# openmm/NNPOps

Measured on AMD Instinct MI355X. Metric: AEV+forces evaluations/sec (ANI-2x symmetry functions, energy+gradient), 10k-atom periodic box, higher is better.
Workload: dtype f32

## Files before the change

### nnpops_amd/csrc/ani.hip

```cpp
#include <algorithm>
#include <cmath>
#include <cstdlib>
#include <cstring>
#include <vector>

#include "ani_kernels.h"
#include "ani_fallback_kernels.h"
#include "ani_angular_mfma.h"
#include "ani_angular_bwd.h"
#include "ani_angular_generic.h"
#include "ani_radial_bwd.h"
#include "ani_build_forward.h"
#include "ani_box_grad.h"
#include "host_common.h"

using namespace nnpops;

constexpr int kRbwdLatencyAtoms = 8192;
constexpr int kFuseAtoms = 4096;
struct nnpops_ani {
    AniParams hp{};
    AngularConsts ac{};
    AniParams* d_params = nullptr;
    int device = 0;
    hipStream_t stream = nullptr;
    int nfrp = 0, nfzp = 0;
    int algorithm = 0;
    int32_t* d_species = nullptr;
    int2* d_segment = nullptr;
    float4* d_nbr = nullptr;
    int* d_cnt_pos = nullptr;
    float4* d_recA = nullptr;
    float4* d_recB = nullptr;
    int* d_ids = nullptr;
// ... 3 lines not shown
    int* d_bucket_offsets = nullptr;
    bool chunked_forward = true;
    int forward_kernel = 2;
    bool generic = false;
    bool mfma_ok = false;
    bool fwd_identity = false;
    int fwd_chunk = 192;
    bool fwd_chunk_forced = false;
    int fwd_waves_per_atom = 2;
    bool backward_forced = false;
    bool fwd_uniform = false;
    bool fwd_grid = true;
    bool bwd_literal = true;
    bool fwd_literal = false;
    int fuse_forward = -1;
    bool rbwd_lanes = true;
    int scatter_mode = -1;
    bool scatter_now = false;
    bool last_fused_build = false;
    int last_bwd_mode = -1;
    int last_radial_lanes = -1;
    int last_tile = -1;
    int last_compact = -1;
    bool fine_grid = true;
    bool fwd_row_via_lds = true;
    int fwd_occ = 7;
    bool fwd_dynamic = false;
    int nstreams = 1;
    hipStream_t side[3] = {nullptr, nullptr, nullptr};
    hipEvent_t ev_fork = nullptr, ev_join[3] = {nullptr, nullptr, nullptr};
// ... 5 lines not shown
    int fwd_atoms_per_group = 1;
    int* d_cnt_a = nullptr;
    int* d_cnt_ro = nullptr;
    double* d_box_partials = nullptr;
    int* d_status = nullptr;
    int* h_status = nullptr;
    int* h_status_dev = nullptr;
    int check_stamp = 0;
    bool check_pending = false;
    CellGrid* d_grid = nullptr;
    int* d_cell_count = nullptr;
    int* d_cell_start = nullptr;
    int* d_atom_cell = nullptr;
    int* d_atom_rank = nullptr;
    int* d_sorted_cell = nullptr;
    int* d_tile_total = nullptr;
    int* d_unsorted_atom = nullptr;
    int* d_sorted_atom = nullptr;
    float4* d_sorted_pos = nullptr;
    int max_cells = 0;
    int* d_hist = nullptr;
    int* d_bins = nullptr;
    int bin_cap = 64;
    bool cells_disabled = false;
    int cap = 0;
    bool cap_fitted = false;
    int cap_angular = 0;
    int tile = 32;
    bool compact_bwd = false;
    bool computed = false;
// ... 304 lines not shown
        h->last_bwd_mode = 1;
        if (lb > 64 * 1024) NNPOPS_HIP_TRY(hipFuncSetAttribute((const void*)k, hipFuncAttributeMaxDynamicSharedMemorySize, (int)lb));
        hipLaunchKernelGGL(k, dim3(N), dim3(64), lb, sp.stream, h->d_params, h->ac, h->cap, h->cap_angular, h->cap_angular, h->d_recA, h->d_recB, h->d_tri,
                           h->d_cnt_a, h->d_cnt_ro, g, h->ld_angular, h->d_leg_force, h->d_centre_force, h->d_ids, nullptr, 0, h->hp.NB, (int)lb, nullptr, 0, N, 0);
    }
    NNPOPS_HIP_TRY(hipGetLastError());
    return NNPOPS_OK;
}

int dispatch_angular(nnpops_ani* h, bool forward, const float* g, float* out, const Span& sp) {
    KernelTimer timer(h, forward ? NNPOPS_ANI_K_ANGULAR_FWD : NNPOPS_ANI_K_ANGULAR_BWD, sp.stream);
    if (h->generic) return h->hp.torchani ? launch_generic<true>(h, forward, g, out, sp) : launch_generic<false>(h, forward, g, out, sp);
    return h->hp.torchani ? dispatch_factors<true>(h, forward, g, out, sp) : dispatch_factors<false>(h, forward, g, out, sp);
}

int fused_chunk(const nnpops_ani* h) {
    return forward_chunk(h, (size_t)h->cap_angular * 2 * sizeof(float4) + (size_t)triples_capacity(h->cap_angular) * sizeof(int) + 64, 12 * sizeof(float));
}

bool build_forward_fused(const nnpops_ani* h, const float* angular) {
    const bool want = h->fuse_forward < 0 ? h->hp.N <= kFuseAtoms : h->fuse_forward != 0;
    return want && !h->generic && h->forward_kernel == 2 && h->fwd_waves_per_atom == 2 && h->nfrp == 8 && h->nfzp == 4 &&
           h->nstreams == 1 && h->fwd_identity && h->ld_angular % 4 == 0 && ((uintptr_t)angular & 15) == 0 &&
           build_forward_lds_bytes<8, 4>(h->cap, h->cap_angular, h->hp.S, h->hp.NB, fused_chunk(h)) <= 160 * 1024;
}

template <bool TA>
int launch_build_forward(nnpops_ani* h, const BuildInputs& in, const BuildOutputs& out, float* angular, const Span& sp) {
    int tri_offset = 0;
    const int CH = fused_chunk(h);
    const size_t lds = (build_forward_lds_bytes<8, 4>(h->cap, h->cap_angular, h->hp.S, h->hp.NB, CH, &tri_offset) + 15) & ~(size_t)15;
    const int vec_ok = 1 | (h->store_mode << 1) | (h->fwd_row_via_lds ? 8 : 0);
    const bool uni = h->fwd_uniform && h->fwd_grid && h->hp.nFR == 8 && h->hp.nFZ == 4;
    const bool dyn = h->fwd_dynamic && h->fwd_row_via_lds && h->hp.NB <= 63 && h->hp.NB * h->hp.nA <= CH * 12;
    auto k = h->fwd_occ == 6 ? ani_build_forward<TA, 8, 4, 6>
           : dyn ? (uni ? ani_build_forward<TA, 8, 4, 7, 1, true> : ani_build_forward<TA, 8, 4, 7, 0, true>)
           : uni ? ani_build_forward<TA, 8, 4, 7, 1> : ani_build_forward<TA, 8, 4, 7>;
    if (uni && h->fwd_literal && h->fwd_occ != 6) k = dyn ? ani_build_forward<TA, 8, 4, 7, 2, true> : ani_build_forward<TA, 8, 4, 7, 2>;
    if (lds > 64 * 1024) NNPOPS_HIP_TRY(hipFuncSetAttribute((const void*)k, hipFuncAttributeMaxDynamicSharedMemorySize, (int)lds));
    hipLaunchKernelGGL(k, dim3(sp.nw), dim3(128), lds, sp.stream, h->d_params, in, out, h->cap, h->cap_angular, CH, angular,
                       h->ld_angular, vec_ok, tri_offset, sp.w0, sp.nw);
    NNPOPS_HIP_TRY(hipGetLastError());
    return NNPOPS_OK;
}

bool pair_backward_fits(const nnpops_ani* h) {
// ... 52 lines not shown
    NNPOPS_REQUIRE(radial_cutoff > 0 && angular_cutoff > 0, "cutoffs must be positive");
    NNPOPS_REQUIRE(angular_cutoff <= radial_cutoff,
                   "angular cutoff (%g) must not exceed the radial cutoff (%g): angular neighbours are drawn from the radial scan "
                   "(reference CpuANISymmetryFunctions.cpp:129-135)", angular_cutoff, radial_cutoff);
    NNPOPS_REQUIRE(num_radial > 0 && num_radial <= kMaxRadialFns, "num_radial must be in [1, %d]", kMaxRadialFns);
    NNPOPS_REQUIRE(num_angular > 0 && num_angular <= kMaxAngularFns, "num_angular must be in [1, %d]", kMaxAngularFns);
    NNPOPS_REQUIRE(atom_species && radial_eta_rs && angular_eta_rs_zeta_ths, "NULL parameter array");
    for (int i = 0; i < num_atoms; i++)
        NNPOPS_REQUIRE(atom_species[i] >= 0 && atom_species[i] < num_species, "atom_species[%d] = %d is outside [0, %d)", i,
                       atom_species[i], num_species);
    int ndev = 0;
    if (hipGetDeviceCount(&ndev) != hipSuccess || ndev == 0) return fail(NNPOPS_ERR_NO_DEVICE, "no HIP device available");
    NNPOPS_REQUIRE(device >= 0 && device < ndev, "device %d out of range (have %d)", device, ndev);

    nnpops_ani* h = new nnpops_ani();
    AniParams& hp = h->hp;
    hp.N = num_atoms; hp.S = num_species; hp.nR = num_radial; hp.nA = num_angular;
    hp.NB = num_species * (num_species + 1) / 2;
    hp.periodic = periodic != 0; hp.torchani = torchani != 0;
    hp.rcr = radial_cutoff; hp.rca = angular_cutoff;
    hp.rcr2 = radial_cutoff * radial_cutoff; hp.rca2 = angular_cutoff * angular_cutoff;
    hp.radial_scale = torchani ? 0.25f : 1.0f;
    hp.inv_rcr = 1.0f / radial_cutoff; hp.inv_rca = 1.0f / angular_cutoff;
    hp.kp_shift = 0;
    while ((1 << hp.kp_shift) < num_radial) hp.kp_shift++;
    hp.angle_damp = torchani ? 0.95f : 1.0f;
    for (int k = 0; k < num_radial; k++) {
        hp.rad_eta[k] = radial_eta_rs[2 * k];
        hp.rad_rs[k] = radial_eta_rs[2 * k + 1];
        hp.rad_c[k] = -radial_eta_rs[2 * k] * kLog2e;
// ... 61 lines not shown
            for (size_t b = 0; b < live.size(); b++)
                for (int p = 0; p < hp.fwd_split; p++) hp.fwd_slot_bucket[b * hp.fwd_split + p] = live[b];
        }
        for (int c = 0; c < kMaxAngularFns; c++) hp.m_of_c[c] = -1;
        h->fwd_identity = num_angular == h->nfrp * h->nfzp;
        for (int m = 0; m < num_angular; m++) {
            hp.m_of_c[hp.c_of_m[m]] = m;
            if (hp.c_of_m[m] != m) h->fwd_identity = false;
        }
        hp.fwd_zero_shift = 0;
        while ((4 << hp.fwd_zero_shift) < num_angular && hp.fwd_zero_shift < 6) hp.fwd_zero_shift++;
        h->fwd_identity = h->fwd_identity && num_angular <= 256;
        h->forward_kernel = h->mfma_ok ? 2 : -1;
        if (const char* e = std::getenv("NNPOPS_ANI_FWD_CHUNK")) { h->fwd_chunk = std::min(512, std::max(64, (std::atoi(e) + 15) / 16 * 16)); h->fwd_chunk_forced = true; }
        if (const char* e = std::getenv("NNPOPS_ANI_FUSE")) h->fuse_forward = std::atoi(e) != 0 ? 1 : 0;
        if (const char* e = std::getenv("NNPOPS_ANI_LPT")) h->lpt = std::atoi(e);
        if (const char* e = std::getenv("NNPOPS_ANI_CELL_ATOMS")) h->cell_atoms = std::max(1, std::atoi(e));
        if (const char* e = std::getenv("NNPOPS_ANI_RBWD")) h->rbwd_lanes = std::atoi(e) != 0;
        if (const char* e = std::getenv("NNPOPS_ANI_SCATTER")) h->scatter_mode = std::atoi(e) != 0 ? 1 : 0;
        if (const char* e = std::getenv("NNPOPS_ANI_FINE_GRID")) h->fine_grid = std::atoi(e) != 0;
        if (const char* e = std::getenv("NNPOPS_ANI_FWD_ROWLDS")) h->fwd_row_via_lds = std::atoi(e) != 0;
        if (const char* e = std::getenv("NNPOPS_ANI_FWD_OCC")) h->fwd_occ = std::atoi(e);
        {
            std::vector<double> frac(num_species, 0.0);
            for (int i = 0; i < num_atoms; i++) frac[atom_species[i]] += 1.0 / num_atoms;
            double fmax = 0;
            for (int a = 0; a < num_species; a++)
                for (int b = a; b < num_species; b++) fmax = std::max(fmax, frac[a] * frac[b] * (a == b ? 1.0 : 2.0));
            h->fwd_dynamic = h->mfma_ok && 32.0 * fmax / hp.fwd_split > 3.0;
        }
// ... 25 lines not shown
    if (periodic && (rc = dev_alloc(&h->d_box_partials, (size_t)9 * ani_box_blocks(num_atoms)))) return cleanup(rc);
    if ((rc = alloc_rows(h))) return cleanup(rc);
    h->max_cells = num_atoms + 4096;
    if ((rc = dev_alloc(&h->d_grid, 1))) return cleanup(rc);
    if ((rc = dev_alloc(&h->d_cell_count, (size_t)h->max_cells))) return cleanup(rc);
    if ((rc = dev_alloc(&h->d_cell_start, (size_t)h->max_cells + 1))) return cleanup(rc);
    if (const char* e = std::getenv("NNPOPS_CELL_BIN_CAP")) h->bin_cap = std::max(4, std::atoi(e) & ~3);
    if (periodic && num_atoms <= kBinnedAtoms) {
        if ((rc = dev_alloc(&h->d_hist, (size_t)kHistWords))) return cleanup(rc);
        if ((rc = dev_alloc(&h->d_bins, (size_t)kBinnedCells * h->bin_cap))) return cleanup(rc);
        if (hipMemset(h->d_hist, 0, sizeof(int) * kHistWords) != hipSuccess) return cleanup(fail(NNPOPS_ERR_HIP, "memset failed"));
    }
    if ((rc = dev_alloc(&h->d_atom_cell, (size_t)num_atoms))) return cleanup(rc);
    if ((rc = dev_alloc(&h->d_atom_rank, (size_t)num_atoms))) return cleanup(rc);
    if ((rc = dev_alloc(&h->d_sorted_cell, (size_t)num_atoms))) return cleanup(rc);
    if ((rc = dev_alloc(&h->d_tile_total, (size_t)h->max_cells / kScanTile + 2))) return cleanup(rc);
    if ((rc = dev_alloc(&h->d_sorted_atom, (size_t)num_atoms))) return cleanup(rc);
    if ((rc = dev_alloc(&h->d_work_order, (size_t)num_atoms))) return cleanup(rc);
    if ((rc = dev_alloc(&h->d_class_tile, (size_t)num_atoms))) return cleanup(rc);
    if (hipMemset(h->d_class_tile, 255, (size_t)num_atoms) != hipSuccess) return cleanup(fail(NNPOPS_ERR_HIP, "memset failed"));
    hp.class_tile = h->d_class_tile;
    if (const char* e = std::getenv("NNPOPS_ANI_BWD_CLASSES")) h->bwd_by_class = std::atoi(e) != 0;
    if (const char* e = std::getenv("NNPOPS_ANI_BWD_CLASS_MIN")) h->bwd_class_min = std::max(0, std::atoi(e));
    if (const char* e = std::getenv("NNPOPS_ANI_BWD_CLASS_ATOMS")) h->bwd_class_atoms = std::max(0, std::atoi(e));
    if ((rc = dev_alloc(&h->d_unsorted_atom, (size_t)num_atoms))) return cleanup(rc);
    if ((rc = dev_alloc(&h->d_sorted_pos, (size_t)num_atoms))) return cleanup(rc);
    if ((rc = dev_alloc(&h->d_bucket_offsets, (size_t)num_atoms * (hp.NB + 1)))) return cleanup(rc);
    hp.bucket_offsets = h->d_bucket_offsets;
    if (hipMemset(h->d_bucket_offsets, 0, sizeof(int) * (size_t)num_atoms * (hp.NB + 1)) != hipSuccess)
        return cleanup(fail(NNPOPS_ERR_HIP, "memset failed"));
// ... 35 lines not shown
        hipMemset(h->d_cnt_a, 0, sizeof(int) * num_atoms) != hipSuccess ||
        hipMemset(h->d_cnt_ro, 0, sizeof(int) * num_atoms) != hipSuccess || hipMemset(h->d_cnt_pos, 0, sizeof(int) * num_atoms) != hipSuccess)
        return cleanup(fail(NNPOPS_ERR_HIP, "parameter upload failed: %s", hipGetErrorString(hipGetLastError())));
    *out = h;
    return NNPOPS_OK;
}

int nnpops_ani_destroy(nnpops_ani_t h) {
    if (!h) return NNPOPS_OK;
    DeviceGuard guard(h->device);
    dev_free(h->d_params); dev_free(h->d_species); dev_free(h->d_segment);
    dev_free(h->d_nbr); dev_free(h->d_recA); dev_free(h->d_recB); dev_free(h->d_tri); dev_free(h->d_cnt_a); dev_free(h->d_cnt_ro); dev_free(h->d_cnt_pos); dev_free(h->d_status); dev_free(h->d_box_partials);
    dev_free(h->d_ids); dev_free(h->d_leg_force); dev_free(h->d_centre_force); dev_free(h->d_bucket_offsets);
    dev_free(h->d_hist); dev_free(h->d_bins);
    dev_free(h->d_grid); dev_free(h->d_cell_count); dev_free(h->d_cell_start); dev_free(h->d_atom_cell);
    dev_free(h->d_atom_rank); dev_free(h->d_sorted_cell); dev_free(h->d_tile_total); dev_free(h->d_sorted_atom); dev_free(h->d_work_order); dev_free(h->d_class_tile); dev_free(h->d_unsorted_atom); dev_free(h->d_sorted_pos);
    for (int q = 0; q < 3; q++) {
        if (h->side[q]) (void)hipStreamDestroy(h->side[q]);
        if (h->ev_join[q]) (void)hipEventDestroy(h->ev_join[q]);
    }
    if (h->ev_fork) (void)hipEventDestroy(h->ev_fork);
    if (h->h_status) (void)hipHostFree(h->h_status);
    for (int k = 0; k < NNPOPS_ANI_NUM_KERNELS; k++) {
        for (hipEvent_t e : h->ev_start[k]) (void)hipEventDestroy(e);
        for (hipEvent_t e : h->ev_stop[k]) (void)hipEventDestroy(e);
    }
    delete h;
    return NNPOPS_OK;
}

int nnpops_ani_set_stream(nnpops_ani_t h, void* stream) {
// ... 51 lines not shown
    DeviceGuard guard(h->device);
    if (!guard.ok) return fail(NNPOPS_ERR_HIP, "cannot select device %d", h->device);
    const int N = h->hp.N;
    const bool per = h->hp.periodic;

    const int lds_bw = (int)((builder_lds_bytes(h->cap, h->hp.S, h->hp.NB) + 15) & ~(size_t)15);
    const int wpg_b = waves_per_group(lds_bw);
    const size_t lds_b = (size_t)lds_bw * wpg_b;
    const dim3 ablock(64 * wpg_b);
    const bool use_cells = !h->d_segment && (h->algorithm == 2 || (h->algorithm == 0 && N >= h->cell_atoms && !h->cells_disabled));
    h->last_used_cells = use_cells;
    if (use_cells) {
        KernelTimer timer(h, NNPOPS_ANI_K_CELL_GRID);
        const CellBuffers cb{h->d_grid, h->d_cell_count, h->d_cell_start, h->d_atom_cell, h->d_atom_rank,
                             h->d_unsorted_atom, h->d_sorted_atom, h->d_sorted_pos, h->max_cells,
                             h->d_hist, h->d_bins, h->bin_cap, h->fine_grid ? 1 : 0, h->d_sorted_cell, h->d_tile_total};
        launch_cell_build(h->stream, N, positions, box, per, h->hp.rcr, h->d_species, cb);
    }
    h->can_split = !h->generic && h->forward_kernel == 2 && h->backward_kernel >= 1 &&
                   pair_backward_fits(h);
    Span spans[4];
    const int nspans = make_spans(h, spans);
    int rc = fork_streams(h, spans, nspans);
    if (rc != NNPOPS_OK) return rc;
    for (int q = 0; q < nspans; q++) {
        const Span& sp = spans[q];
        const dim3 sgrid(div_up(sp.nw, wpg_b));
        h->last_fused_build = build_forward_fused(h, angular);
        if (h->last_fused_build) {
            KernelTimer timer(h, NNPOPS_ANI_K_NEIGHBORS, sp.stream);
            KernelTimer merged_timer(h, NNPOPS_ANI_K_NEIGHBORS, sp.stream, true);
            const BuildInputs in{box, h->d_grid, h->d_cell_start, h->d_sorted_cell, h->d_sorted_pos, h->d_hist, positions, h->d_species,
                                 h->d_segment, use_cells ? 1 : 0, per ? 1 : 0};
            const BuildOutputs out{h->d_nbr, h->d_recA, h->d_recB, h->d_ids, h->d_tri, h->d_cnt_a, h->d_cnt_ro, h->d_cnt_pos, h->d_status, radial, h->ld_radial};
            rc = h->hp.torchani ? launch_build_forward<true>(h, in, out, angular, sp) : launch_build_forward<false>(h, in, out, angular, sp);
            if (rc != NNPOPS_OK) return rc;
            continue;
        }
        KernelTimer merged_timer(h, NNPOPS_ANI_K_NEIGHBORS, sp.stream, true);
        {
        KernelTimer timer(h, NNPOPS_ANI_K_NEIGHBORS, sp.stream);
        if (use_cells) {
            if (per)
                hipLaunchKernelGGL(ani_neighbors_cells<true>, sgrid, ablock, lds_b, sp.stream, h->d_params, box, h->d_grid,
                                   h->d_cell_start, h->d_sorted_cell, h->d_sorted_pos, h->d_nbr, h->cap, h->cap_angular, h->d_recA,
                                   h->d_recB, h->d_ids, h->d_tri, h->d_cnt_a, h->d_cnt_ro, h->d_cnt_pos, h->d_status, radial, h->ld_radial, lds_bw, h->d_hist,
                                   sp.w0, sp.nw);
            else
// ... 332 lines not shown
    if (!guard.ok) return fail(NNPOPS_ERR_HIP, "cannot select device %d", h->device);
    NNPOPS_HIP_TRY(hipMemcpyAsync(value, h->d_status + kStatOverflow, sizeof(int32_t), hipMemcpyDeviceToHost, h->stream));
    NNPOPS_HIP_TRY(hipStreamSynchronize(h->stream));
    return NNPOPS_OK;
}

int nnpops_ani_describe(nnpops_ani_t h, char* text, int capacity) {
    NNPOPS_REQUIRE(h != nullptr && text != nullptr && capacity > 0, "NULL argument");
    const bool uni = h->fwd_uniform && h->hp.nFR == h->nfrp && h->hp.nFZ == h->nfzp;
    const bool shape2x = h->nfrp == 8 && h->nfzp == 4;
    std::snprintf(text, (size_t)capacity,
                  "forward=%s backward=%d generic=%d uniform=%d grid=%d literal=%d dynamic_quads=%d fused_build=%d cap=%d cap_angular=%d "
                  "chunk=%d classes=%d cells=%d scatter=%d row_major_walk=%d bwd_mode=%d radial_bwd=%s tile=%d compact=%d",
                  h->forward_kernel == 2 ? "mfma" : h->forward_kernel == 1 ? "chunked" : "merge", h->backward_kernel, (int)h->generic,
                  (int)uni, (int)(uni && h->fwd_grid), (int)(uni && h->fwd_grid && shape2x && h->fwd_literal), (int)h->fwd_dynamic,
                  (int)(h->computed ? h->last_fused_build : (h->fuse_forward < 0 ? h->hp.N <= kFuseAtoms : h->fuse_forward != 0)), h->cap, h->cap_angular,
                  h->generic ? h->fwd_chunk : forward_chunk(h, (size_t)h->cap_angular * 2 * sizeof(float4), (size_t)(h->nfrp + h->nfzp) * sizeof(float)),
                  (int)h->bwd_classes.size(), (int)h->last_used_cells,
                  (int)h->scatter_now, h->hp.tri_row_major,
                  h->last_bwd_mode, h->last_radial_lanes < 0 ? "none" : h->last_radial_lanes ? "lanes" : "rows", h->last_tile, h->last_compact);
    return NNPOPS_OK;
}

int nnpops_ani_enable_timing(nnpops_ani_t h, int enable) {
    NNPOPS_REQUIRE(h != nullptr, "NULL handle");
    h->timing_mask = enable == 1 ? ~0u : (unsigned)enable >> 1;
    for (int k = 0; k < NNPOPS_ANI_NUM_KERNELS; k++) { h->ev_used[k] = 0; h->timing_seen[k] = 0; }
    return NNPOPS_OK;
}

int nnpops_ani_set_timing_stride(nnpops_ani_t h, int every) {
// ... 54 lines not shown
```

### nnpops_amd/csrc/ani_build_forward.h

```cpp
#pragma once

#include "ani_angular_mfma.h"

namespace nnpops {

template <int NFRP, int NFZP>
__host__ __device__ inline size_t build_forward_lds_bytes(int cap, int capA, int S, int NB, int CH, int* tri_offset = nullptr) {
    const size_t recs = (size_t)capA * 2 * sizeof(float4);
    const size_t staging = (size_t)(CH + 1) * (NFRP + NFZP) * sizeof(float) + 64 * sizeof(int);
    const size_t builder = ((builder_lds_bytes(cap, S, NB) + 15) & ~(size_t)15) + 32;
    const size_t mid = ((staging > builder ? staging : builder) + 15) & ~(size_t)15;
    if (tri_offset) *tri_offset = (int)(recs + mid);
    return recs + mid + (size_t)triples_capacity(capA) * sizeof(int);
}

struct BuildInputs {
    const float* box;
    const CellGrid* grid;
    const int* cell_start;
    const int* sorted_cell;
    const float4* sorted_pos;
    int* cell_hist;
    const float* pos;
    const int* species;
    const int2* segment;
    int use_cells, periodic;
};

struct BuildOutputs {
    float4* nbr;
    float4 *recA, *recB;
    int *ids, *tri, *cnt_a, *cnt_ro, *cnt_pos, *status;
    float* radial;
    int ld_radial;
};

template <bool TORCHANI, int NFRP, int NFZP, int OCC, int UNI = 0, bool DYN = false>
__global__ __launch_bounds__(128, OCC) void ani_build_forward(const AniParams* __restrict__ P, BuildInputs in, BuildOutputs out, int cap,
                                                              int capA, int CH, float* __restrict__ angular, int ld_angular,
                                                              int vec_ok, int tri_offset, int w0, int nw) {
    extern __shared__ __attribute__((aligned(16))) char lds_raw[];
    const int role = __builtin_amdgcn_readfirstlane(wave_in_group());
    const int lane = lane_id();
    float4* recA_l = (float4*)lds_raw;
    float4* recB_l = recA_l + capA;
    float4* stage = recB_l + capA;
    float* rscratch = (float*)(stage + cap);
    int* groups = (int*)(rscratch + 3 * cap + 64 * P->S);
    const AtomGroups G = carve_groups(groups, P->S, P->NB);
    int* shared = groups + ((group_ints(P->S, P->NB, cap) + 3) & ~(size_t)3);
    int* tri_l = (int*)(lds_raw + tri_offset);
    clear_cell_histogram(in.use_cells ? in.cell_hist : nullptr);

    const float rcr2 = P->rcr2, rca2 = P->rca2;
    Box b{};
    if (in.periodic) b = load_box(in.box);
    CellGrid g{};
    if (in.use_cells) g = *in.grid;

    {
        const int w = blockIdx.x;
        const int slot_id = w0 + w;
        int i = slot_id;
        float4 me = make_float4(0.f, 0.f, 0.f, 0.f);
        const bool void_grid = in.use_cells && !g.ok;
        if (in.use_cells && !void_grid) {
            me = in.sorted_pos[slot_id];
            i = __float_as_int(me.w) & kIdMask;
        } else if (!in.use_cells) {
            me = make_float4(in.pos[3 * i], in.pos[3 * i + 1], in.pos[3 * i + 2], 0.f);
        }
        if (role == 0) {
            int na = 0, nro = 0;
            if (void_grid) {
                if (lane == 0 && slot_id == 0) atomicOr(&out.status[kStatOverflow], g.bin_overflow ? 6 : 2);
            } else if (in.use_cells) {
                const int c = in.sorted_cell[slot_id];
                int cx, cy, cz;
                split_cell(g, c, cx, cy, cz);
                const WideStencil st = gather_wide_stencil(g, in.cell_start, cx, cy, cz);
// ... 49 lines not shown
        const int na_raw = shared[0], nro_raw = shared[1];
        clamp_counts(na_raw, nro_raw, cap, capA, n, nro_c);
        if (!void_grid) {
            if (role == 1) {
                flush_row(out.nbr + (size_t)slot_id * cap, stage, cap, na_raw, nro_raw);
                radial_forward_from_lds(P, stage, cap, n, nro_c, rscratch, out.radial + (size_t)i * out.ld_radial);
            } else {
                finalize_angular(P, stage, n, out.recA + (size_t)i * capA, out.recB + (size_t)i * capA, out.ids + (size_t)i * capA, capA,
                                 out.tri + (size_t)i * triples_capacity(capA), P->bucket_offsets + (size_t)i * (P->NB + 1), G,
                                 recA_l, recB_l, tri_l);
            }
        }
        __syncthreads();
        MfmaForward<TORCHANI, NFRP, NFZP, 2, UNI, DYN> F;
        F.init(P, capA, CH, vec_ok, angular, ld_angular, lds_raw, role);
        F.atom(i, n, [&](int t) { return tri_l[t]; }, [&](int bk) { return G.boff[bk]; }, [&]() { F.write_zero_record(); });
    }
}

}
```

### nnpops_amd/csrc/celllist.h

```cpp
#pragma once

#include "device_common.h"

namespace nnpops {

constexpr int kTagShift = 24;
constexpr int kIdMask = (1 << kTagShift) - 1;

struct CellGrid {
    int nx, ny, nz, ncells;
    int periodic;
    int m;
    int ok;
    int bin_overflow;
    float ox, oy, oz;
    float ixx, iyy, izz;
    float bx, cx, cy;
};

__device__ __forceinline__ void cell_of(const CellGrid& g, float x, float y, float z, int& cx, int& cy, int& cz) {
    float sz = (z - g.oz) * g.izz;
    float sy = ((y - g.oy) - sz * g.cy) * g.iyy;
    float sx = ((x - g.ox) - sy * g.bx - sz * g.cx) * g.ixx;
    if (g.periodic) {
// ... 166 lines not shown
        }
    if ((int)blockIdx.x == ntiles - 1 && threadIdx.x == 0) cell_start[ncells] = off + tile_total[blockIdx.x];
}

static __global__ void fill_cells(int N, const CellGrid* __restrict__ grid, const int* __restrict__ cell_start,
                           const int* __restrict__ atom_cell, const int* __restrict__ atom_rank,
                           int* __restrict__ sorted_atom) {
    const int i = blockIdx.x * blockDim.x + threadIdx.x;
    if (i >= N || !grid->ok) return;
    sorted_atom[cell_start[atom_cell[i]] + atom_rank[i]] = i;
}

static __global__ void order_cells(int N, const float* __restrict__ pos, const CellGrid* __restrict__ grid,
                            const int* __restrict__ cell_start, const int* __restrict__ atom_cell,
                            const int* __restrict__ unsorted_atom, const int* __restrict__ tag,
                            int* __restrict__ sorted_atom, float4* __restrict__ sorted_pos, int* __restrict__ sorted_cell) {
    const int i = blockIdx.x * blockDim.x + threadIdx.x;
    if (i >= N || !grid->ok) return;
    const int c = atom_cell[i];
    const int lo = cell_start[c], hi = cell_start[c + 1];
    int rank = 0;
    for (int a = lo; a < hi; a++) rank += unsorted_atom[a] < i;
    sorted_atom[lo + rank] = i;
    if (sorted_cell) sorted_cell[lo + rank] = c;
    const int packed = i | (tag ? (tag[i] << kTagShift) : 0);
    sorted_pos[lo + rank] = make_float4(pos[3 * i], pos[3 * i + 1], pos[3 * i + 2], __int_as_float(packed));
}

constexpr int kBinnedAtoms = 65536;
constexpr int kPairsBinnedAtoms = 200000, kPairsBinCap = 128;
constexpr int kBinnedCells = 8192;
constexpr int kBinnedThreads = 256;

constexpr int kHistWords = kBinnedCells + 1;

__device__ __forceinline__ int bin_one_atom(int i, int N, const CellGrid& g, float x, float y, float z, int* __restrict__ hist,
                                            int* __restrict__ bins, int bin_cap) {
    if (i >= N || !g.ok) return -1;
    int cx, cy, cz;
    cell_of(g, x, y, z, cx, cy, cz);
    const int c = (cz * g.ny + cy) * g.nx + cx;
    const int r = atomicAdd(&hist[c], 1);
    if (r < bin_cap) bins[(size_t)c * bin_cap + r] = i;
    else hist[kBinnedCells] = 1;
    return c;
}

template <int T>
__device__ __forceinline__ void order_block(int N, CellGrid* __restrict__ grid, const float* __restrict__ pos,
                                            const int* __restrict__ tag, const int* __restrict__ hist, const int* __restrict__ bins,
                                            int bin_cap, const int* __restrict__ atom_cell, int* __restrict__ cell_start,
                                            int* __restrict__ sorted_atom, float4* __restrict__ sorted_pos,
                                            int* __restrict__ sorted_cell, int* s_start, int* wave_tot) {
    const int tid = threadIdx.x, lane = tid & 63, wave = tid >> 6;
    const int i = blockIdx.x * T + tid, ic = min(i, N - 1);
    const CellGrid g = *grid;
    const int c = atom_cell[ic];
    const float px = pos[3 * ic], py = pos[3 * ic + 1], pz = pos[3 * ic + 2];
    const int packed = ic | (tag ? (tag[ic] << kTagShift) : 0);
    const int overflowed = hist[kBinnedCells];
    constexpr int PER = kBinnedCells / T;
    int mine[PER];
#pragma unroll
    for (int q = 0; q < PER; q++) mine[q] = hist[q * T + tid];
    const int4* bin4 = reinterpret_cast<const int4*>(bins + (size_t)min(max(c, 0), kBinnedCells - 1) * bin_cap);
    const int4 first = bin4[0], second = bin_cap >= 8 ? bin4[1] : make_int4(0, 0, 0, 0);
    if (!g.ok) return;
    if (overflowed != 0) {
// ... 13 lines not shown
    __syncthreads();
    int run = incl - sum;
    for (int w = 0; w < wave; w++) run += wave_tot[w];
    for (int q = c0; q < c1; q++) { const int v = s_start[q]; s_start[q] = run; run += v; }
    if (tid == T - 1) s_start[ncells] = run;
    __syncthreads();
    for (int q = blockIdx.x * T + tid; q <= ncells; q += gridDim.x * T) cell_start[q] = s_start[q];

    if (i >= N) return;
    const int lo = s_start[c], n = s_start[c + 1] - lo;
    auto below = [&](const int4& v, int k) { return (k < n && v.x < i) + (k + 1 < n && v.y < i) + (k + 2 < n && v.z < i) + (k + 3 < n && v.w < i); };
    int rank = below(first, 0) + below(second, 4);
    for (int k = 8; k < n; k += 4) rank += below(bin4[k >> 2], k);
    sorted_atom[lo + rank] = i;
    if (sorted_cell) sorted_cell[lo + rank] = c;
    sorted_pos[lo + rank] = make_float4(px, py, pz, __int_as_float(packed));
}

static __global__ __launch_bounds__(kBinnedThreads) void bin_atoms(int N, const float* __restrict__ pos,
                                                                   const float* __restrict__ box, float cutoff, int max_cells,
                                                                   CellGrid* __restrict__ grid, int* __restrict__ hist,
                                                                   int* __restrict__ bins, int bin_cap,
                                                                   int* __restrict__ atom_cell, int fine) {
    __shared__ CellGrid g;
    const int i = blockIdx.x * kBinnedThreads + threadIdx.x;
    const int ic = min(i, N - 1);
    const float x = pos[3 * ic], y = pos[3 * ic + 1], z = pos[3 * ic + 2];
    if (threadIdx.x == 0) {
        g = decide_grid(1, box, nullptr, nullptr, cutoff, min(max_cells, kBinnedCells), fine);
        if (blockIdx.x == 0) *grid = g;
    }
    __syncthreads();
    const int c = bin_one_atom(i, N, g, x, y, z, hist, bins, bin_cap);
    if (c >= 0) atom_cell[i] = c;
}

template <int T>
static __global__ __launch_bounds__(T) void order_binned(int N, const float* __restrict__ pos,
                                                                      const int* __restrict__ tag, CellGrid* __restrict__ grid,
                                                                      const int* __restrict__ hist,
                                                                      const int* __restrict__ bins, int bin_cap,
                                                                      const int* __restrict__ atom_cell, int* __restrict__ cell_start,
                                                                      int* __restrict__ sorted_atom, float4* __restrict__ sorted_pos,
                                                                      int* __restrict__ sorted_cell) {
    __shared__ int s_start[kBinnedCells + 1];
    __shared__ int wave_tot[T / 64];
    order_block<T>(N, grid, pos, tag, hist, bins, bin_cap, atom_cell, cell_start, sorted_atom, sorted_pos, sorted_cell, s_start, wave_tot);
}

constexpr int kStencilRanges = 18;
struct Stencil {
    int pre[kStencilRanges];
    int delta;
    int total;
};

__device__ __forceinline__ Stencil gather_stencil(const CellGrid& g, const int* __restrict__ cell_start, int cx, int cy, int cz) {
    const int lane = lane_id();
    int begin = 0, end = 0;
    if (lane < kStencilRanges) {
        const int pair = lane >> 1, sub = lane & 1;
        int z = cz + pair / 3 - 1, y = cy + pair % 3 - 1;
// ... 187 lines not shown
}

struct CellBuffers {
    CellGrid* grid;
    int *cell_count, *cell_start;
    int *atom_cell, *atom_rank;
    int *unsorted_atom, *sorted_atom;
    float4* sorted_pos;
    int max_cells;
    int* hist = nullptr;
    int* bins = nullptr;
    int bin_cap = 0;
    int fine = 0;
    int* sorted_cell = nullptr;
    int* tile_total = nullptr;
};

static inline bool cell_build_is_binned(int N, bool periodic, const CellBuffers& b) {
    return periodic && b.hist != nullptr && b.bins != nullptr;
}

static inline void launch_cell_build(hipStream_t stream, int N, const float* pos, const float* box, bool periodic, float cutoff,
                                     const int* tag, const CellBuffers& b) {
    const int tb = 256, nb = (N + tb - 1) / tb;
    if (cell_build_is_binned(N, periodic, b)) {
        hipLaunchKernelGGL(bin_atoms, dim3(nb), dim3(kBinnedThreads), 0, stream, N, pos, box, cutoff, b.max_cells, b.grid, b.hist, b.bins,
                           b.bin_cap, b.atom_cell, b.fine);
        hipLaunchKernelGGL(order_binned<kBinnedThreads>, dim3(nb), dim3(kBinnedThreads), 0, stream, N, pos, tag, b.grid, b.hist, b.bins, b.bin_cap,
                           b.atom_cell, b.cell_start, b.sorted_atom, b.sorted_pos, b.sorted_cell);
        return;
    }
    hipLaunchKernelGGL(grid_setup, dim3(periodic ? 32 : 1), dim3(256), 0, stream, N, pos, box, (int)periodic, cutoff, b.max_cells, b.grid, b.cell_count, b.fine);
    hipLaunchKernelGGL(assign_cells, dim3(nb), dim3(tb), 0, stream, N, pos, b.grid, b.cell_count, b.atom_cell, b.atom_rank);
    if (b.max_cells <= kScanTile || b.tile_total == nullptr) {
        hipLaunchKernelGGL(scan_cells, dim3(1), dim3(1024), 0, stream, b.grid, b.cell_count, b.cell_start, (int*)nullptr);
    } else {
        const int ntiles = (b.max_cells + kScanTile - 1) / kScanTile;
        hipLaunchKernelGGL(scan_cells, dim3(ntiles), dim3(1024), 0, stream, b.grid, b.cell_count, b.cell_start, b.tile_total);
        hipLaunchKernelGGL(add_tile_offsets, dim3(ntiles), dim3(1024), 0, stream, b.grid, b.tile_total, b.cell_start);
    }
    hipLaunchKernelGGL(fill_cells, dim3(nb), dim3(tb), 0, stream, N, b.grid, b.cell_start, b.atom_cell, b.atom_rank, b.unsorted_atom);
    hipLaunchKernelGGL(order_cells, dim3(nb), dim3(tb), 0, stream, N, pos, b.grid, b.cell_start, b.atom_cell, b.unsorted_atom, tag,
                       b.sorted_atom, b.sorted_pos, b.sorted_cell);
}

template <typename F>
__device__ __forceinline__ void for_each_stencil_range(const CellGrid& g, const int* __restrict__ cell_start, int cx,
                                                       int cy, int cz, F&& f) {
    for (int dz = -1; dz <= 1; dz++) {
        int z = cz + dz;
        if (g.periodic) z = (z + g.nz) % g.nz;
        else if (z < 0 || z >= g.nz) continue;
        for (int dy = -1; dy <= 1; dy++) {
            int y = cy + dy;
            if (g.periodic) y = (y + g.ny) % g.ny;
            else if (y < 0 || y >= g.ny) continue;
            const int rowbase = (z * g.ny + y) * g.nx;
            int x0 = cx - 1, x1 = cx + 1;
// ... 18 lines not shown
```

Measured before the change: 12380.

## Extend fused build-forward to large systems by spilling triples to global memory

The fixed atom-count threshold for fusing neighbor build with the angular forward kernel is replaced by a residency-based plan computed from the CU count and LDS footprint. When the triples list would not fit in LDS, a variant keeps triples in global memory, which shrinks LDS so more blocks stay resident and lets larger systems such as the 10k-atom box take the fused path. Optionally the fused kernel walks atoms in the load-balanced work order, using a new slot_of map filled during cell ordering. The trade-off is extra global-memory traffic for the triples and a small amount of extra bookkeeping in the cell build.

```diff
diff --git a/nnpops_amd/csrc/ani.hip b/nnpops_amd/csrc/ani.hip
--- a/nnpops_amd/csrc/ani.hip
+++ b/nnpops_amd/csrc/ani.hip
@@ -17,7 +17,6 @@
 using namespace nnpops;
 
 constexpr int kRbwdLatencyAtoms = 8192;
-constexpr int kFuseAtoms = 4096;
 struct nnpops_ani {
     AniParams hp{};
     AngularConsts ac{};
@@ -51,6 +50,9 @@
     bool bwd_literal = true;
     bool fwd_literal = false;
     int fuse_forward = -1;
+    int fuse_tri_lds = -1;
+    int fuse_order = -1;
+    int num_cus = 256;
     bool rbwd_lanes = true;
     int scatter_mode = -1;
     bool scatter_now = false;
@@ -86,6 +88,7 @@
     int* d_atom_cell = nullptr;
     int* d_atom_rank = nullptr;
     int* d_sorted_cell = nullptr;
+    int* d_slot_of = nullptr;
     int* d_tile_total = nullptr;
     int* d_unsorted_atom = nullptr;
     int* d_sorted_atom = nullptr;
@@ -420,22 +423,40 @@
     return h->hp.torchani ? dispatch_factors<true>(h, forward, g, out, sp) : dispatch_factors<false>(h, forward, g, out, sp);
 }
 
-int fused_chunk(const nnpops_ani* h) {
-    return forward_chunk(h, (size_t)h->cap_angular * 2 * sizeof(float4) + (size_t)triples_capacity(h->cap_angular) * sizeof(int) + 64, 12 * sizeof(float));
+int fused_chunk(const nnpops_ani* h, int flags) {
+    const size_t tri = (flags & kFuseTriGlobal) ? 0 : (size_t)triples_capacity(h->cap_angular) * sizeof(int);
+    return forward_chunk(h, (size_t)h->cap_angular * 2 * sizeof(float4) + tri + 64, 12 * sizeof(float));
+}
+
+size_t fused_lds_bytes(const nnpops_ani* h, int flags, int* tri_offset = nullptr) {
+    return build_forward_lds_bytes<8, 4>(h->cap, h->cap_angular, h->hp.S, h->hp.NB, fused_chunk(h, flags), tri_offset, flags);
+}
+
+int fuse_plan(const nnpops_ani* h) {
+    if (h->fuse_forward == 0) return -1;
+    auto resident = [&](int f) { return (long)h->num_cus * (long)std::min<size_t>(16, 128 / ((fused_lds_bytes(h, f) + 1279) / 1280)); };
+    for (int f : {0, (int)kFuseTriGlobal}) {
+        if (h->fuse_tri_lds >= 0 && (h->fuse_tri_lds != 0) != (f == 0)) continue;
+        if (h->hp.N <= resident(f) || (h->fuse_forward > 0 && (f != 0 || h->fuse_tri_lds > 0))) return f;
+    }
+    return -1;
+}
+
+bool fusable(const nnpops_ani* h) {
+    return !h->generic && h->forward_kernel == 2 && h->fwd_waves_per_atom == 2 && h->nfrp == 8 && h->nfzp == 4 && h->nstreams == 1 &&
+           h->fwd_identity;
 }
 
 bool build_forward_fused(const nnpops_ani* h, const float* angular) {
-    const bool want = h->fuse_forward < 0 ? h->hp.N <= kFuseAtoms : h->fuse_forward != 0;
-    return want && !h->generic && h->forward_kernel == 2 && h->fwd_waves_per_atom == 2 && h->nfrp == 8 && h->nfzp == 4 &&
-           h->nstreams == 1 && h->fwd_identity && h->ld_angular % 4 == 0 && ((uintptr_t)angular & 15) == 0 &&
-           build_forward_lds_bytes<8, 4>(h->cap, h->cap_angular, h->hp.S, h->hp.NB, fused_chunk(h)) <= 160 * 1024;
+    const int plan = fusable(h) ? fuse_plan(h) : -1;
+    return plan >= 0 && h->ld_angular % 4 == 0 && ((uintptr_t)angular & 15) == 0 && fused_lds_bytes(h, plan) <= 160 * 1024;
 }
 
 template <bool TA>
 int launch_build_forward(nnpops_ani* h, const BuildInputs& in, const BuildOutputs& out, float* angular, const Span& sp) {
     int tri_offset = 0;
-    const int CH = fused_chunk(h);
-    const size_t lds = (build_forward_lds_bytes<8, 4>(h->cap, h->cap_angular, h->hp.S, h->hp.NB, CH, &tri_offset) + 15) & ~(size_t)15;
+    const int CH = fused_chunk(h, in.flags);
+    const size_t lds = (fused_lds_bytes(h, in.flags, &tri_offset) + 15) & ~(size_t)15;
     const int vec_ok = 1 | (h->store_mode << 1) | (h->fwd_row_via_lds ? 8 : 0);
     const bool uni = h->fwd_uniform && h->fwd_grid && h->hp.nFR == 8 && h->hp.nFZ == 4;
     const bool dyn = h->fwd_dynamic && h->fwd_row_via_lds && h->hp.NB <= 63 && h->hp.NB * h->hp.nA <= CH * 12;
@@ -518,6 +539,7 @@
     NNPOPS_REQUIRE(device >= 0 && device < ndev, "device %d out of range (have %d)", device, ndev);
 
     nnpops_ani* h = new nnpops_ani();
+    if (hipDeviceGetAttribute(&h->num_cus, hipDeviceAttributeMultiprocessorCount, device) != hipSuccess || h->num_cus <= 0) h->num_cus = 256;
     AniParams& hp = h->hp;
     hp.N = num_atoms; hp.S = num_species; hp.nR = num_radial; hp.nA = num_angular;
     hp.NB = num_species * (num_species + 1) / 2;
@@ -609,6 +631,8 @@
         h->forward_kernel = h->mfma_ok ? 2 : -1;
         if (const char* e = std::getenv("NNPOPS_ANI_FWD_CHUNK")) { h->fwd_chunk = std::min(512, std::max(64, (std::atoi(e) + 15) / 16 * 16)); h->fwd_chunk_forced = true; }
         if (const char* e = std::getenv("NNPOPS_ANI_FUSE")) h->fuse_forward = std::atoi(e) != 0 ? 1 : 0;
+        if (const char* e = std::getenv("NNPOPS_ANI_FUSE_TRI_LDS")) h->fuse_tri_lds = std::atoi(e) != 0 ? 1 : 0;
+        if (const char* e = std::getenv("NNPOPS_ANI_FUSE_ORDER")) h->fuse_order = std::atoi(e) != 0 ? 1 : 0;
         if (const char* e = std::getenv("NNPOPS_ANI_LPT")) h->lpt = std::atoi(e);
         if (const char* e = std::getenv("NNPOPS_ANI_CELL_ATOMS")) h->cell_atoms = std::max(1, std::atoi(e));
         if (const char* e = std::getenv("NNPOPS_ANI_RBWD")) h->rbwd_lanes = std::atoi(e) != 0;
@@ -664,6 +688,8 @@
     if ((rc = dev_alloc(&h->d_atom_cell, (size_t)num_atoms))) return cleanup(rc);
     if ((rc = dev_alloc(&h->d_atom_rank, (size_t)num_atoms))) return cleanup(rc);
     if ((rc = dev_alloc(&h->d_sorted_cell, (size_t)num_atoms))) return cleanup(rc);
+    if ((rc = dev_alloc(&h->d_slot_of, (size_t)num_atoms))) return cleanup(rc);
+    if (hipMemset(h->d_slot_of, 0, sizeof(int) * (size_t)num_atoms) != hipSuccess) return cleanup(fail(NNPOPS_ERR_HIP, "memset failed"));
     if ((rc = dev_alloc(&h->d_tile_total, (size_t)h->max_cells / kScanTile + 2))) return cleanup(rc);
     if ((rc = dev_alloc(&h->d_sorted_atom, (size_t)num_atoms))) return cleanup(rc);
     if ((rc = dev_alloc(&h->d_work_order, (size_t)num_atoms))) return cleanup(rc);
@@ -729,7 +755,7 @@
     dev_free(h->d_ids); dev_free(h->d_leg_force); dev_free(h->d_centre_force); dev_free(h->d_bucket_offsets);
     dev_free(h->d_hist); dev_free(h->d_bins);
     dev_free(h->d_grid); dev_free(h->d_cell_count); dev_free(h->d_cell_start); dev_free(h->d_atom_cell);
-    dev_free(h->d_atom_rank); dev_free(h->d_sorted_cell); dev_free(h->d_tile_total); dev_free(h->d_sorted_atom); dev_free(h->d_work_order); dev_free(h->d_class_tile); dev_free(h->d_unsorted_atom); dev_free(h->d_sorted_pos);
+    dev_free(h->d_atom_rank); dev_free(h->d_sorted_cell); dev_free(h->d_slot_of); dev_free(h->d_tile_total); dev_free(h->d_sorted_atom); dev_free(h->d_work_order); dev_free(h->d_class_tile); dev_free(h->d_unsorted_atom); dev_free(h->d_sorted_pos);
     for (int q = 0; q < 3; q++) {
         if (h->side[q]) (void)hipStreamDestroy(h->side[q]);
         if (h->ev_join[q]) (void)hipEventDestroy(h->ev_join[q]);
@@ -811,7 +837,7 @@
         KernelTimer timer(h, NNPOPS_ANI_K_CELL_GRID);
         const CellBuffers cb{h->d_grid, h->d_cell_count, h->d_cell_start, h->d_atom_cell, h->d_atom_rank,
                              h->d_unsorted_atom, h->d_sorted_atom, h->d_sorted_pos, h->max_cells,
-                             h->d_hist, h->d_bins, h->bin_cap, h->fine_grid ? 1 : 0, h->d_sorted_cell, h->d_tile_total};
+                             h->d_hist, h->d_bins, h->bin_cap, h->fine_grid ? 1 : 0, h->d_sorted_cell, h->d_tile_total, h->d_slot_of};
         launch_cell_build(h->stream, N, positions, box, per, h->hp.rcr, h->d_species, cb);
     }
     h->can_split = !h->generic && h->forward_kernel == 2 && h->backward_kernel >= 1 &&
@@ -827,8 +853,12 @@
         if (h->last_fused_build) {
             KernelTimer timer(h, NNPOPS_ANI_K_NEIGHBORS, sp.stream);
             KernelTimer merged_timer(h, NNPOPS_ANI_K_NEIGHBORS, sp.stream, true);
-            const BuildInputs in{box, h->d_grid, h->d_cell_start, h->d_sorted_cell, h->d_sorted_pos, h->d_hist, positions, h->d_species,
-                                 h->d_segment, use_cells ? 1 : 0, per ? 1 : 0};
+            const int flags = fuse_plan(h);
+            const bool walk_order = sp.ang_order == h->d_work_order && h->work_order_valid &&
+                                    (h->fuse_order < 0 ? (flags & kFuseTriGlobal) != 0 : h->fuse_order != 0);
+            const BuildInputs in{box, h->d_grid, h->d_cell_start, h->d_sorted_cell, h->d_sorted_pos, h->d_hist,
+                                 walk_order ? h->d_work_order : nullptr, h->d_slot_of, positions, h->d_species,
+                                 h->d_segment, use_cells ? 1 : 0, per ? 1 : 0, flags};
             const BuildOutputs out{h->d_nbr, h->d_recA, h->d_recB, h->d_ids, h->d_tri, h->d_cnt_a, h->d_cnt_ro, h->d_cnt_pos, h->d_status, radial, h->ld_radial};
             rc = h->hp.torchani ? launch_build_forward<true>(h, in, out, angular, sp) : launch_build_forward<false>(h, in, out, angular, sp);
             if (rc != NNPOPS_OK) return rc;
@@ -1191,7 +1221,7 @@
                   "chunk=%d classes=%d cells=%d scatter=%d row_major_walk=%d bwd_mode=%d radial_bwd=%s tile=%d compact=%d",
                   h->forward_kernel == 2 ? "mfma" : h->forward_kernel == 1 ? "chunked" : "merge", h->backward_kernel, (int)h->generic,
                   (int)uni, (int)(uni && h->fwd_grid), (int)(uni && h->fwd_grid && shape2x && h->fwd_literal), (int)h->fwd_dynamic,
-                  (int)(h->computed ? h->last_fused_build : (h->fuse_forward < 0 ? h->hp.N <= kFuseAtoms : h->fuse_forward != 0)), h->cap, h->cap_angular,
+                  (int)(h->computed ? h->last_fused_build : (fusable(h) && fuse_plan(h) >= 0)), h->cap, h->cap_angular,
                   h->generic ? h->fwd_chunk : forward_chunk(h, (size_t)h->cap_angular * 2 * sizeof(float4), (size_t)(h->nfrp + h->nfzp) * sizeof(float)),
                   (int)h->bwd_classes.size(), (int)h->last_used_cells,
                   (int)h->scatter_now, h->hp.tri_row_major,
diff --git a/nnpops_amd/csrc/ani_build_forward.h b/nnpops_amd/csrc/ani_build_forward.h
--- a/nnpops_amd/csrc/ani_build_forward.h
+++ b/nnpops_amd/csrc/ani_build_forward.h
@@ -4,14 +4,16 @@
 
 namespace nnpops {
 
+enum { kFuseTriGlobal = 1 };
+
 template <int NFRP, int NFZP>
-__host__ __device__ inline size_t build_forward_lds_bytes(int cap, int capA, int S, int NB, int CH, int* tri_offset = nullptr) {
+__host__ __device__ inline size_t build_forward_lds_bytes(int cap, int capA, int S, int NB, int CH, int* tri_offset = nullptr, int flags = 0) {
     const size_t recs = (size_t)capA * 2 * sizeof(float4);
     const size_t staging = (size_t)(CH + 1) * (NFRP + NFZP) * sizeof(float) + 64 * sizeof(int);
     const size_t builder = ((builder_lds_bytes(cap, S, NB) + 15) & ~(size_t)15) + 32;
     const size_t mid = ((staging > builder ? staging : builder) + 15) & ~(size_t)15;
-    if (tri_offset) *tri_offset = (int)(recs + mid);
-    return recs + mid + (size_t)triples_capacity(capA) * sizeof(int);
+    if (tri_offset) *tri_offset = (flags & kFuseTriGlobal) ? -1 : (int)(recs + mid);
+    return recs + mid + ((flags & kFuseTriGlobal) ? 0 : (size_t)triples_capacity(capA) * sizeof(int));
 }
 
 struct BuildInputs {
@@ -21,10 +23,13 @@
     const int* sorted_cell;
     const float4* sorted_pos;
     int* cell_hist;
+    const int* order;
+    const int* slot_of;
     const float* pos;
     const int* species;
     const int2* segment;
     int use_cells, periodic;
+    int flags;
 };
 
 struct BuildOutputs {
@@ -49,7 +54,7 @@
     int* groups = (int*)(rscratch + 3 * cap + 64 * P->S);
     const AtomGroups G = carve_groups(groups, P->S, P->NB);
     int* shared = groups + ((group_ints(P->S, P->NB, cap) + 3) & ~(size_t)3);
-    int* tri_l = (int*)(lds_raw + tri_offset);
+    int* tri_l = tri_offset >= 0 ? (int*)(lds_raw + tri_offset) : nullptr;
     clear_cell_histogram(in.use_cells ? in.cell_hist : nullptr);
 
     const float rcr2 = P->rcr2, rca2 = P->rca2;
@@ -60,10 +65,14 @@
 
     {
         const int w = blockIdx.x;
-        const int slot_id = w0 + w;
+        const bool void_grid = in.use_cells && !g.ok;
+        int slot_id = w0 + w;
         int i = slot_id;
+        if (in.order && !void_grid) {
+            i = in.order[slot_id];
+            slot_id = in.use_cells ? in.slot_of[i] : i;
+        }
         float4 me = make_float4(0.f, 0.f, 0.f, 0.f);
-        const bool void_grid = in.use_cells && !g.ok;
         if (in.use_cells && !void_grid) {
             me = in.sorted_pos[slot_id];
             i = __float_as_int(me.w) & kIdMask;
@@ -143,7 +152,9 @@
         __syncthreads();
         MfmaForward<TORCHANI, NFRP, NFZP, 2, UNI, DYN> F;
         F.init(P, capA, CH, vec_ok, angular, ld_angular, lds_raw, role);
-        F.atom(i, n, [&](int t) { return tri_l[t]; }, [&](int bk) { return G.boff[bk]; }, [&]() { F.write_zero_record(); });
+        const int* tri_g = out.tri + (size_t)i * triples_capacity(capA);
+        F.atom(i, n, [&](int t) { return tri_l ? tri_l[t] : __hip_atomic_load(tri_g + t, __ATOMIC_RELAXED, __HIP_MEMORY_SCOPE_WORKGROUP); },
+               [&](int bk) { return G.boff[bk]; }, [&]() { F.write_zero_record(); });
     }
 }
 
diff --git a/nnpops_amd/csrc/celllist.h b/nnpops_amd/csrc/celllist.h
--- a/nnpops_amd/csrc/celllist.h
+++ b/nnpops_amd/csrc/celllist.h
@@ -204,7 +204,8 @@
 static __global__ void order_cells(int N, const float* __restrict__ pos, const CellGrid* __restrict__ grid,
                             const int* __restrict__ cell_start, const int* __restrict__ atom_cell,
                             const int* __restrict__ unsorted_atom, const int* __restrict__ tag,
-                            int* __restrict__ sorted_atom, float4* __restrict__ sorted_pos, int* __restrict__ sorted_cell) {
+                            int* __restrict__ sorted_atom, float4* __restrict__ sorted_pos, int* __restrict__ sorted_cell,
+                            int* __restrict__ slot_of) {
     const int i = blockIdx.x * blockDim.x + threadIdx.x;
     if (i >= N || !grid->ok) return;
     const int c = atom_cell[i];
@@ -213,6 +214,7 @@
     for (int a = lo; a < hi; a++) rank += unsorted_atom[a] < i;
     sorted_atom[lo + rank] = i;
     if (sorted_cell) sorted_cell[lo + rank] = c;
+    if (slot_of) slot_of[i] = lo + rank;
     const int packed = i | (tag ? (tag[i] << kTagShift) : 0);
     sorted_pos[lo + rank] = make_float4(pos[3 * i], pos[3 * i + 1], pos[3 * i + 2], __int_as_float(packed));
 }
@@ -241,7 +243,8 @@
                                             const int* __restrict__ tag, const int* __restrict__ hist, const int* __restrict__ bins,
                                             int bin_cap, const int* __restrict__ atom_cell, int* __restrict__ cell_start,
                                             int* __restrict__ sorted_atom, float4* __restrict__ sorted_pos,
-                                            int* __restrict__ sorted_cell, int* s_start, int* wave_tot) {
+                                            int* __restrict__ sorted_cell, int* s_start, int* wave_tot,
+                                            int* __restrict__ slot_of = nullptr) {
     const int tid = threadIdx.x, lane = tid & 63, wave = tid >> 6;
     const int i = blockIdx.x * T + tid, ic = min(i, N - 1);
     const CellGrid g = *grid;
@@ -285,6 +288,7 @@
     for (int k = 8; k < n; k += 4) rank += below(bin4[k >> 2], k);
     sorted_atom[lo + rank] = i;
     if (sorted_cell) sorted_cell[lo + rank] = c;
+    if (slot_of) slot_of[i] = lo + rank;
     sorted_pos[lo + rank] = make_float4(px, py, pz, __int_as_float(packed));
 }
 
@@ -313,10 +317,10 @@
                                                                       const int* __restrict__ bins, int bin_cap,
                                                                       const int* __restrict__ atom_cell, int* __restrict__ cell_start,
                                                                       int* __restrict__ sorted_atom, float4* __restrict__ sorted_pos,
-                                                                      int* __restrict__ sorted_cell) {
+                                                                      int* __restrict__ sorted_cell, int* __restrict__ slot_of) {
     __shared__ int s_start[kBinnedCells + 1];
     __shared__ int wave_tot[T / 64];
-    order_block<T>(N, grid, pos, tag, hist, bins, bin_cap, atom_cell, cell_start, sorted_atom, sorted_pos, sorted_cell, s_start, wave_tot);
+    order_block<T>(N, grid, pos, tag, hist, bins, bin_cap, atom_cell, cell_start, sorted_atom, sorted_pos, sorted_cell, s_start, wave_tot, slot_of);
 }
 
 constexpr int kStencilRanges = 18;
@@ -534,6 +538,7 @@
     int fine = 0;
     int* sorted_cell = nullptr;
     int* tile_total = nullptr;
+    int* slot_of = nullptr;
 };
 
 static inline bool cell_build_is_binned(int N, bool periodic, const CellBuffers& b) {
@@ -547,7 +552,7 @@
         hipLaunchKernelGGL(bin_atoms, dim3(nb), dim3(kBinnedThreads), 0, stream, N, pos, box, cutoff, b.max_cells, b.grid, b.hist, b.bins,
                            b.bin_cap, b.atom_cell, b.fine);
         hipLaunchKernelGGL(order_binned<kBinnedThreads>, dim3(nb), dim3(kBinnedThreads), 0, stream, N, pos, tag, b.grid, b.hist, b.bins, b.bin_cap,
-                           b.atom_cell, b.cell_start, b.sorted_atom, b.sorted_pos, b.sorted_cell);
+                           b.atom_cell, b.cell_start, b.sorted_atom, b.sorted_pos, b.sorted_cell, b.slot_of);
         return;
     }
     hipLaunchKernelGGL(grid_setup, dim3(periodic ? 32 : 1), dim3(256), 0, stream, N, pos, box, (int)periodic, cutoff, b.max_cells, b.grid, b.cell_count, b.fine);
@@ -561,7 +566,7 @@
     }
     hipLaunchKernelGGL(fill_cells, dim3(nb), dim3(tb), 0, stream, N, b.grid, b.cell_start, b.atom_cell, b.atom_rank, b.unsorted_atom);
     hipLaunchKernelGGL(order_cells, dim3(nb), dim3(tb), 0, stream, N, pos, b.grid, b.cell_start, b.atom_cell, b.unsorted_atom, tag,
-                       b.sorted_atom, b.sorted_pos, b.sorted_cell);
+                       b.sorted_atom, b.sorted_pos, b.sorted_cell, b.slot_of);
 }
 
 template <typename F>
```

Result: no change. 12310 (-0.6%).
